# XChenZ/havatar

Hardware: AMD Instinct MI355X
Metric: rendered frames/sec @512^2, 64 samples/ray (higher is better)
Workload: dtype f32 emulated, full-width operands: every operand = hi + lo fp16 + tail (= the fp32 value itself, >= 24 significant bits); the three leading partial products on v_mfma_f32_32x32x16_f16, the three terms of order 2^-22 (hi.tail, tail.hi, lo.lo) on block-scaled 4-/6-bit v_mfma_scale_f32_32x32x64_f8f6f4

## Files before the change

### havatar_amd/_lib.py

```python
import ctypes as C
import os

from . import switches

_HERE = os.path.dirname(os.path.abspath(__file__))
LIB_PATH = os.path.join(_HERE, "lib", "libhavatar_hip.so")

HAV_F32, HAV_F16, HAV_BF16, HAV_F64 = 0, 1, 2, 3
HAV_MLP_SPLIT_BF16, HAV_MLP_F32, HAV_MLP_SPLIT_F16, HAV_MLP_SPLIT_F16_MX = 0, 1, 2, 3
ABI_VERSION = 8
HAV_FLAG_PAIR_KERNEL, HAV_FLAG_FINE_CACHE, HAV_FLAG_FINE_RECOMPUTE, HAV_FLAG_NO_FP16_GUARD = 1, 2, 4, 8
HAV_STATUS_FP16_FALLBACK = 1


class HavRenderParams(C.Structure):
    _fields_ = [("B", C.c_int32), ("R", C.c_int32), ("ray_stride", C.c_int32), ("S_c", C.c_int32),
                ("S_f", C.c_int32), ("perturb", C.c_int32), ("noise_std", C.c_float),
                ("plane_res", C.c_int32), ("plane_ch", C.c_int32), ("vol_res", C.c_int32),
                ("nerf_scale", C.c_float * 3), ("nerf_trans", C.c_float * 3),
                ("skin_scale", C.c_float * 3), ("skin_trans", C.c_float * 3),
                ("seed", C.c_uint64), ("rng_offset", C.c_uint64), ("mlp_mode", C.c_int32), ("flags", C.c_int32),
                ("rng_counter", C.c_void_p), ("workspace", C.c_void_p), ("workspace_bytes", C.c_uint64),
                ("dbg_zfine", C.c_void_p), ("status", C.c_void_p), ("grid_blocks", C.c_int32), ("reserved0", C.c_int32)]

# ... 65 lines not shown
    L.hav_triplane_gather_bwd.restype = i32
    L.hav_field_inputs_fwd.argtypes = [vp, C.POINTER(HavFieldParams), vp, vp, vp, vp, vp]
    L.hav_field_inputs_fwd.restype = i32
    L.hav_field_inputs_fwd_bf16.argtypes = [vp, C.POINTER(HavFieldParams), vp, vp, vp, vp, vp]
    L.hav_field_inputs_fwd_bf16.restype = i32
    L.hav_field_inputs_bwd.argtypes = [vp, vp, vp, C.POINTER(HavFieldParams), vp, vp, vp, vp, vp]
    L.hav_field_inputs_bwd.restype = i32
    L.hav_field_inputs_bwd_rows.argtypes = [vp, vp, vp, C.POINTER(HavFieldParams), vp, vp, vp, vp, i32, vp]
    L.hav_field_inputs_bwd_rows.restype = i32
    L.hav_field_inputs_bwd_fixed.argtypes = [vp, vp, vp, vp, vp, C.POINTER(HavFieldParams), vp, vp, vp, vp, vp]
    L.hav_field_inputs_bwd_fixed.restype = i32
    L.hav_field_inputs_bwd_fixed_scratch_bytes.argtypes = [C.POINTER(HavFieldParams)]
    L.hav_field_inputs_bwd_fixed_scratch_bytes.restype = i64
    L.hav_composite_fwd.argtypes = [vp] * 9 + [i64, i32, i32, i32, vp]
    L.hav_composite_fwd.restype = i32
    L.hav_composite_bwd.argtypes = [vp] * 10 + [i64, i32, i32, i32, vp]
    L.hav_composite_bwd.restype = i32
    for name, args in (("hav_composite_long_fwd", [vp] * 9 + [i64, i32, i32, i32, vp]),
                       ("hav_composite_long_bwd", [vp] * 10 + [i64, i32, i32, i32, vp]),
                       ("hav_composite_long_bwd_form", [vp] * 10 + [i64, i32, i32, i32, i32, vp]),
                       ("hav_haar_down2", [vp] * 5 + [f32, i32, i32, i32, i32, vp]),
                       ("hav_s2_image_loss_blocks", [i32, i32]),
                       ("hav_s2_image_loss_fwd", [vp, vp, vp] + [i64] * 4 + [vp] + [i64] * 3 + [vp] * 4 + [i32, i32, i32, vp]),
                       ("hav_s2_image_loss_bwd", [vp, vp] + [i64] * 4 + [vp, vp, vp] + [i64] * 4 + [vp] + [i64] * 3 + [vp] * 4
                        + [i32, i32, i32, i32, vp]),
                       ("hav_lpips_head_blocks", [i32] * 4),
                       ("hav_lpips_head_fwd", [vp] * 5 + [i32] * 4 + [vp]),
                       ("hav_lpips_head_bwd", [vp] * 6 + [i32] * 4 + [vp]),
                       ("hav_relu_mask_bwd", [vp] * 4 + [i32, i32, i64, vp]),
                       ("hav_image_metrics_blocks", [i32] * 4),
                       ("hav_image_metrics_f32", [vp] * 5 + [i32] * 4 + [f32, vp]),
                       ("hav_image_metrics_u8", [vp] * 5 + [i32] * 3 + [vp]),
                       ("hav_ssim_grad_blocks", [i32] * 4),
                       ("hav_ssim_loss_bwd_f32", [vp] * 5 + [i32] * 4 + [f32, vp])):
        try:
            fn = getattr(L, name)
        except AttributeError:
            raise HavatarLibraryError(f"{path} does not export {name}: it was built from older sources; rebuild it with "
                                      "`python -m havatar_amd.build --force`") from None
        fn.argtypes, fn.restype = args, (i64 if name.endswith("_blocks") else i32)
    L.hav_resample_depths.argtypes = [vp] * 5 + [i64, i32, i32, vp]
    L.hav_resample_depths.restype = i32
    L.hav_equal_linear_fwd.argtypes = [vp] * 4 + [C.c_float, C.c_float, i32, i32, i32, vp]
    L.hav_equal_linear_fwd.restype = i32
    L.hav_equal_linear_bwd.argtypes = [vp] * 6 + [C.c_float, C.c_float, i32, i32, i32, vp]
    L.hav_equal_linear_bwd.restype = i32
    L.hav_mlp_blob_bytes.restype = i64
    L.hav_mlp_pack.argtypes = [vp, C.POINTER(HavMlpWeights), vp]
    L.hav_mlp_pack.restype = i32
    for fn in (L.hav_haar_dwt, L.hav_haar_idwt):
        fn.argtypes = [vp, vp, vp, i32, i32, i32, i32, vp]
        fn.restype = i32
    L.hav_style_mlp.argtypes = [vp, vp, vp, i32, i32, i32, i32, f32, f32, vp]
    L.hav_style_mlp.restype = i32
    L.hav_haar_up2.argtypes = [vp, vp, vp, vp, vp, i32, i32, i32, i32, vp]
    L.hav_haar_up2.restype = i32
    L.hav_conv3x3_wgrad_scratch_bytes.argtypes = [i32] * 5
    L.hav_conv3x3_wgrad_scratch_bytes.restype = i64
    L.hav_conv3x3_wgrad.argtypes = [vp, vp, vp, vp, vp, vp, i32, i32, i32, i32, i32, vp]
    L.hav_conv3x3_wgrad.restype = i32
    L.hav_gemm_packed_bytes.argtypes = [i32, i32]
    L.hav_gemm_packed_bytes.restype = i64
    L.hav_gemm_pack.argtypes = [vp, vp, i32, i32, f32, vp]
    L.hav_gemm_pack.restype = i32
    L.hav_gemm_split.argtypes = [vp, vp, vp, vp, vp, i32, i32, i32, i32, vp]
    L.hav_gemm_split.restype = i32
    L.hav_upconv_finish.argtypes = [vp] * 7 + [f32, f32, i32, i32, i32, i32, i32, i32, vp]
# ... 106 lines not shown
```

### havatar_amd/build.py

```python
import os
import subprocess
import sys

from . import switches

HERE = os.path.dirname(os.path.abspath(__file__))
CSRC = os.path.join(HERE, "csrc")
LIBDIR = os.path.join(HERE, "lib")
LIB = os.path.join(LIBDIR, "libhavatar_hip.so")
SOURCES = ["hav_ops.hip", "hav_render.hip", "hav_train.hip", "hav_mlp_train.hip", "hav_conv.hip", "hav_conv3d.hip", "hav_decoder.hip",
           "hav_composite_long.hip", "hav_stage2.hip", "hav_s2_loss.hip", "hav_lpips.hip", "hav_metrics.hip", "hav_ssim_loss.hip"]
HEADERS = ["hav_common.h", os.path.join("..", "..", "include", "havatar.h")]
FLAGS = ["--offload-arch=gfx950", "-O3", "-std=c++17", "-fPIC", "-Wall", "-Wno-unused-function", "-Wno-unused-variable"]
BUILD_INFO = os.path.join(LIBDIR, "BUILD_INFO.json")
TESTED_HIPCC = ("HIP version: 7.2.26015-fc0010cf6a",
                "AMD clang version 22.0.0git (https://github.com/RadeonOpenCompute/llvm-project roc-7.2.0 26014 7b800a19466229b8479a78de19143dc33c3ab9b5)")


def hipcc_version(hipcc):
    out = subprocess.run([hipcc, "--version"], stdout=subprocess.PIPE, stderr=subprocess.STDOUT, check=False).stdout.decode(errors="replace")
    return tuple(ln.strip() for ln in out.splitlines()[:2])


def check_compiler(hipcc):
    ver = hipcc_version(hipcc)
    tested = ver == TESTED_HIPCC
    if not tested:
        msg = ("hipcc differs from the compiler this library's kernels were validated with:\n  found  %s\n  tested %s\n"
               "Re-run tools/stress_production.py and the -m gpu determinism tests on a GPU with the new build." % (ver, TESTED_HIPCC))
        if switches.off("HAVATAR_REQUIRE_TESTED_HIPCC"):
            raise RuntimeError(msg)
        import warnings
        warnings.warn(msg, RuntimeWarning, stacklevel=2)
    return ver, tested


def _stale():
    if not os.path.exists(LIB):
        return True
    t = os.path.getmtime(LIB)
    return any(os.path.getmtime(os.path.join(CSRC, f)) > t for f in SOURCES + HEADERS)


def build_info():
    import json
# ... 38 lines not shown
```

### havatar_amd/csrc/hav_render.hip

```cpp
#include "hav_common.h"
#include <stdio.h>
#include <stdlib.h>
#include <string.h>
#include <atomic>

#define HAV_HID 128
#define HAV_PC 64
#define HAV_IN (2 * HAV_PC + 48)
#define KPE_STEPS 24
#define K2_STEPS (HAV_HID / 2)
#define OFF_W1PE 0
#define OFF_W2 (OFF_W1PE + KPE_STEPS * 4 * 64)
#define OFF_W4 (OFF_W2 + K2_STEPS * 4 * 64)
#define OFF_WFT (OFF_W4 + K2_STEPS * 2 * 4)
#define LDS_FLOATS (OFF_WFT + HAV_HID * 64)
#define OFF_B1 LDS_FLOATS
#define OFF_B2 (OFF_B1 + 128)
#define OFF_B4 (OFF_B2 + 128)
#define OFF_BF (OFF_B4 + 4)
#define OFF_W1F (OFF_BF + 64)
#define OFF_WFF (OFF_W1F + 2 * 128 * 64)
#define OFF_A1S (OFF_WFF + K2_STEPS * 2 * 64)
#define OFF_A2S (OFF_A1S + 3 * 4 * 3 * 64 * 4)
#define OFF_W4S (OFF_A2S + 8 * 4 * 3 * 64 * 4)
#define LDS3_FLOATS (3 * 4 * 3 * 64 * 4 + 8 * 4 * 3 * 64 * 4 + K2_STEPS * 2 * 4)
#define OFF_A1H (OFF_W4S + K2_STEPS * 2 * 4)
#define OFF_A2H (OFF_A1H + 3 * 4 * 2 * 64 * 4)
#define OFF_W4H (OFF_A2H + 8 * 4 * 2 * 64 * 4)
#define OFF_AFH (OFF_W4H + K2_STEPS * 2 * 4)
#define HAV_TAPPAIR 1
#define HAV_TG 2
#define HAV_TG1 2
#define LDSH_FLOATS (3 * 4 * 2 * 64 * 4 + 8 * 4 * 2 * 64 * 4 + K2_STEPS * 2 * 4 + 8 * 2 * 2 * 64 * 4)
// ... 328 lines not shown

static bool attr_done(std::atomic<unsigned long long>& mask, int& dev)
{
    dev = 0;
    if (hipGetDevice(&dev) != hipSuccess || dev < 0 || dev > 63) dev = 0;
    return (mask.load(std::memory_order_acquire) >> dev) & 1ull;
}

extern "C" int hav_triplane_prepare(float* dst, const float* src_nchw, const void* mlp_blob, int B, int C, int H, int W,
                                    void* stream)
{
    if (!dst || !src_nchw || !mlp_blob || B < 1 || H < 1 || W < 1) return HAV_EINVAL;
    if (C != HAV_PC || (W & ((1 << HAV_TG) - 1)) || (W & ((1 << HAV_TG1) - 1))) return HAV_EUNSUP;
    const int HW = H * W;
    const size_t lds = (64 * 64 + 128 * 65 + 64 * 129) * sizeof(float);
    static std::atomic<unsigned long long> attr_mask{0};
    int dev;
    if (!attr_done(attr_mask, dev)) {
        hipError_t e = hipFuncSetAttribute((const void*)plane_project_kernel, hipFuncAttributeMaxDynamicSharedMemorySize, (int)lds);
        if (e != hipSuccess) return (int)e;
        attr_mask.fetch_or(1ull << dev, std::memory_order_release);
    }
    unsigned int* trailer = reinterpret_cast<unsigned int*>(dst + (size_t)2 * B * HW * 128);
    hipError_t me = hipMemsetAsync(trailer, 0, PREP_TRAILER_WORDS * 4, (hipStream_t)stream);
    if (me != hipSuccess) return (int)me;
    hipLaunchKernelGGL(plane_project_kernel, dim3((HW + 63) / 64, 2 * B), dim3(256), lds, (hipStream_t)stream, dst, src_nchw,
                       (const float*)mlp_blob, HW, trailer);
    HAV_LAUNCH_CHECK();
    hipLaunchKernelGGL(range_verdict_kernel, dim3(1), dim3(128), 0, (hipStream_t)stream, trailer, (const float*)mlp_blob);
    HAV_LAUNCH_CHECK();
    return 0;
}

#define DPP_QUAD_XOR1 0xB1
#define DPP_QUAD_XOR2 0x4E
#define DPP_ROW_SHR(n) (0x110 + (n))
#define DPP_ROW_MIRROR 0x140
#define DPP_ROW_HALF_MIRROR 0x141

template <int CTRL> __device__ __forceinline__ float dpp_mov(float old, float v)
{
    return __int_as_float(__builtin_amdgcn_update_dpp(__float_as_int(old), __float_as_int(v), CTRL, 0xf, 0xf, false));
}
__device__ __forceinline__ float row16_sum(float v)
{
    v += dpp_mov<DPP_QUAD_XOR1>(0.f, v);
    v += dpp_mov<DPP_QUAD_XOR2>(0.f, v);
    v += dpp_mov<DPP_ROW_HALF_MIRROR>(0.f, v);
    v += dpp_mov<DPP_ROW_MIRROR>(0.f, v);
    return v;
}
__device__ __forceinline__ float row16_max(float v)
{
    v = fmaxf(v, dpp_mov<DPP_QUAD_XOR1>(0.f, v));
    v = fmaxf(v, dpp_mov<DPP_QUAD_XOR2>(0.f, v));
    v = fmaxf(v, dpp_mov<DPP_ROW_HALF_MIRROR>(0.f, v));
    v = fmaxf(v, dpp_mov<DPP_ROW_MIRROR>(0.f, v));
    return v;
}
__device__ __forceinline__ float row16_scan_mul(float v)
{
    v *= dpp_mov<DPP_ROW_SHR(1)>(1.f, v);
    v *= dpp_mov<DPP_ROW_SHR(2)>(1.f, v);
    v *= dpp_mov<DPP_ROW_SHR(4)>(1.f, v);
    v *= dpp_mov<DPP_ROW_SHR(8)>(1.f, v);
    return v;
// ... 1723 lines not shown
```

### havatar_amd/model/nerf_model.py

```python
import logging

import torch
import torch.nn as nn

from .network.embedder import get_embedder
from .styleUnet import StyleGAN_zxc
from .. import switches
from ..utils.sh_util import eval_sh
from ..utils.util import create_UniformBoxWarp, sample_from_triplane_new

_MLP_MODE_LOGGED = False


class _SplitKLinear(torch.autograd.Function):

    @staticmethod
    def forward(ctx, x, weight, bias):
        ctx.save_for_backward(x, weight)
        ctx.has_bias = bias is not None
        return torch.nn.functional.linear(x, weight, bias)

    @staticmethod
    def backward(ctx, dy):
        x, weight = ctx.saved_tensors
# ... 16 lines not shown
    return layer(x)


class ConditionalTriplaneNeRFModel_multiRender_split_view(nn.Module):
    def __init__(self, XYZ_bounding, num_encoding_fn_xyz=8, latent_code_dim=32, triPlane_feat_dim=32, rgb_feat_dim=32,
                 triplane_res=256, use_emb=True, enc_mode="split", sh_deg=2, cond_latent=True, cond_c_dim=0):
        super().__init__()
        if enc_mode != "split":
            raise NotImplementedError("only enc_mode='split' is on the hot path (model/nerf_trainer.py:19-26)")
        self.name = "ConditionalTriplaneNeRFModel_multiRender_split_view"
        self.pos_embedder, self.dim_xyz = get_embedder(multires=num_encoding_fn_xyz, input_dims=3, include_input=False)
        self.sh_deg = sh_deg
        self.use_sh = sh_deg >= 1
        include_xyz = self.dim_xyz if use_emb else 0
        self.dim_latent_code = 0 if cond_latent else latent_code_dim
        self.triPlane_feat_dim = triPlane_feat_dim
        self.rgb_feat_dim = rgb_feat_dim * (sh_deg + 1) ** 2
        self.use_emb, self.cond_latent, self.cond_c_dim = use_emb, cond_latent, cond_c_dim
        self.shared_backbone = self.two_head = False
        enc = dict(out_ch=triPlane_feat_dim, out_size=triplane_res, style_dim=latent_code_dim, middle_size=16, zero_latent=False,
                   zero_noise=True, no_skip=True, n_mlp=4, inp_size=256)
        self.XY_gen = StyleGAN_zxc(inp_ch=7, **enc)
        self.YZ_gen = StyleGAN_zxc(inp_ch=13, **enc)
        self.gridwarper = create_UniformBoxWarp(XYZ_bounding)
        self.layers_xyz = nn.ModuleList([nn.Linear(2 * triPlane_feat_dim + self.dim_latent_code + include_xyz, 128), nn.Linear(128, 128)])
        self.fc_alpha = nn.Linear(128, 1)
        self.fc_rgbFeat = nn.Linear(128, 64)
        self.fc_rgb = nn.Linear(64, self.rgb_feat_dim)
        self.relu = torch.nn.functional.relu
        self.triPlane_embeddings = None
        if not cond_latent:
            self.register_buffer("zero_latent", torch.zeros(latent_code_dim, dtype=torch.float32).reshape(1, -1))

    def set_conditional_embedding(self, **cond):
        styles = None
        if "latents" in cond:
            lat = cond["latents"]
            c = cond["cond_c"].reshape(lat.shape[0], -1)
            if self.cond_latent:
                styles = [torch.cat([lat, c], -1)] if self.cond_c_dim > 0 else [lat]
            else:
                styles = [self.zero_latent.expand(lat.shape[0], -1)]
        front, right = cond["front_render_cond"], cond["right_render_cond"]
        left = cond["left_render_cond"].flip(dims=[3])
        if left.shape[1] > 3:
            left = left[:, :-1]
        yz_in = torch.cat([left, right], dim=1)
        if front.is_cuda and not torch.is_grad_enabled() and switches.on("HAVATAR_ENC_STREAMS"):
            cur = torch.cuda.current_stream(front.device)
            side = self.__dict__.get("_side_stream")
            if side is None or side.device != front.device:
                side = self.__dict__["_side_stream"] = torch.cuda.Stream(device=front.device)
            side.wait_stream(cur)
            with torch.cuda.stream(side):
                yz, _ = self.YZ_gen(styles, yz_in)
            xy, _ = self.XY_gen(styles, front)
            cur.wait_stream(side)
            yz.record_stream(cur)
        else:
            xy, _ = self.XY_gen(styles, front)
            yz, _ = self.YZ_gen(styles, yz_in)
        self.triPlane_embeddings = torch.stack([xy, yz], dim=0)

    def sample_pts_triplane_feat(self, batch_pts, bidx=None):
        q = self.gridwarper(batch_pts)
        planes = self.triPlane_embeddings if bidx is None else self.triPlane_embeddings[:, bidx]
        if q.is_cuda and q.dtype == torch.float32 and q.ndim == 3 and planes.ndim == 5 and planes.shape[0] == 2 \
                and switches.on("HAVATAR_HIP_GATHER"):
            from ..native.gather import triplane_gather
            return triplane_gather(q, planes)
        f = sample_from_triplane_new(q, planes, padding_mode="zeros")
        return f.reshape(-1, f.shape[-1] * f.shape[-2])

    def forward(self, inp, pts_feat):
        xyz, dirs = inp[..., :3], inp[..., 3:]
        return self.mlp(torch.cat([pts_feat, self.pos_embedder(xyz)], -1), dirs)

    def mlp(self, x, dirs=None):
        if (x.is_cuda and x.dtype == torch.float32 and x.ndim == 2 and x.shape[1] == 176 and self.sh_deg == 0 and x.shape[0] >= 1024
                and torch.is_grad_enabled() and switches.choice("HAVATAR_TRAIN_MLP") == "bf16"):
            from ..native import mlp_train
            ws = self.mlp_tensors()
            if [tuple(w.shape) for w in ws] == mlp_train._SHAPES:
                global _MLP_MODE_LOGGED
                if not _MLP_MODE_LOGGED:
                    _MLP_MODE_LOGGED = True
                    logging.getLogger("havatar_amd").info(
                        "radiance MLP under autograd: bf16-operand MFMA node (HAVATAR_TRAIN_MLP=bf16; parameter gradients in the 2e-2 "
                        "class of fp32 nn.Linear) -- HAVATAR_TRAIN_MLP=torch keeps the reference's fp32 layers")
                return mlp_train.fused_mlp(x, ws)
        for layer in self.layers_xyz:
            x = self.relu(_linear(layer, x))
        alpha = _linear(self.fc_alpha, x)
        x = _linear(self.fc_rgbFeat, x)
# ... 9 lines not shown
```

### havatar_amd/model/nerf_trainer.py

```python
import numpy as np
import torch
from einops import rearrange

from . import nerf_model
from .. import switches
from .Skinning_Field import Deformation_Field_new
from ..render import RayMarcher
from ..utils.nerf_util import sample_pdf, volume_render_radiance_field
from ..utils.training_util import get_minibatches
from ..utils.util import UniformBoxWarp_new, get_box_warp_param


_warned_wide_sampling = False


def _warn_wide_sampling(widest):
    global _warned_wide_sampling
    if _warned_wide_sampling:
        return
    _warned_wide_sampling = True
    import warnings
    warnings.warn("training with %d samples in a pass: the native compositing kernels hold 64, so this step takes the ATen statement of "
                  "the whole march.  Set HAVATAR_COMPOSITE_LONG=1 to keep it on the native route (up to 128 samples per pass)." % widest,
                  RuntimeWarning, stacklevel=3)


class Trainer(torch.nn.Module):
    def __init__(self, cfg, latent_codes_size=0, freeze_motion=True):
        super().__init__()
        self.cfg = cfg
        e = cfg.experiment
        self.latent_codes = torch.nn.Parameter(torch.zeros(latent_codes_size, e.latent_code_dim)) if latent_codes_size > 0 else None
        self.model_mode = e.model_mode
        latent_code_dim = e.latent_code_dim + (12 if e.cond_pose else 0) + (52 if e.cond_expr else 0)
        bounding = cfg.models.coarse.XYZ_bounding
        self.model_coarse = nerf_model.ConditionalTriplaneNeRFModel_multiRender_split_view(
            XYZ_bounding=bounding, triPlane_feat_dim=64, rgb_feat_dim=3, triplane_res=128, sh_deg=0,
            latent_code_dim=latent_code_dim, cond_c_dim=latent_code_dim - e.latent_code_dim)
        self.render_size, self.gen_size = cfg.models.StyleUnet.inp_size, cfg.models.StyleUnet.out_size
        b = {k: np.asarray(v, dtype=np.float64).copy() for k, v in zip("XYZ", bounding)}
        b["Y"][0] = 0.3 * b["Y"][1]
        scales, trans = get_box_warp_param(b["X"], b["Y"], b["Z"])
        self.headpose_skin_net = Deformation_Field_new(gridwarper=UniformBoxWarp_new(scales=scales, trans=trans))
        if freeze_motion:
            self.headpose_skin_net.requires_grad = False
        self._marcher = None

    def _hip_marcher(self):
        if self._marcher is None:
            gw, sw = self.model_coarse.gridwarper, self.headpose_skin_net.gridwarper
            f = lambda t: t.detach().reshape(3).cpu().tolist()
            self._marcher = RayMarcher(f(gw.scale_factor), f(gw.trans_factor), f(sw.scale_factor), f(sw.trans_factor))
        return self._marcher

    def nerf_forward(self, **inputs):
        cond_c = inputs["inv_head_T"].view(inputs["inv_head_T"].shape[0], -1)
        self.model_coarse.set_conditional_embedding(
            front_render_cond=inputs["front_render_cond"], left_render_cond=inputs["left_render_cond"],
            right_render_cond=inputs["right_render_cond"], latents=inputs["latent_code"], cond_c=cond_c)
        self._planes_dirty = True
        inv_head_T, ray_batch, background_prior = inputs["inv_head_T"], inputs["ray_batch"], inputs["background_prior"]
        mode = inputs["mode"]
        opt = getattr(self.cfg.nerf, mode)
        rd = ray_batch[..., 3:6]
        restore = [rd.shape[:-1] + (-1,), rd.shape[:-1], rd.shape[:-1], rd.shape[:-1]]
        if opt.num_fine > 0:
            restore += restore[:-1]
        if ray_batch.is_cuda:
            rays = ray_batch
        else:
            viewdirs = rd / rd.norm(p=2, dim=-1).unsqueeze(-1)
            rays = torch.cat((ray_batch, viewdirs), dim=-1)
        if self._use_hip(rays):
            self._decline_coarse = bool(inputs.get("_fine_maps_only", False)) and opt.num_fine > 0
            out = list(self.predict_and_render_radiance(mode, rays, background_prior, inv_head_T=inv_head_T))
            self._decline_coarse = False
        else:
            if rays.is_cuda:
                cap = max(switches.integer("HAVATAR_TRAIN_CHUNK_RAYS"), opt.chunksize)
                chunk = min(rays.shape[1], max(cap // rays.shape[0], 1))
            else:
                chunk = opt.chunksize // rays.shape[0]
            rb = get_minibatches(rays, chunksize=chunk, dim=1)
            bg = get_minibatches(background_prior, chunksize=chunk, dim=1) if background_prior is not None else None
            pred = [self.predict_and_render_radiance(mode, r, None if bg is None else bg[i], inv_head_T=inv_head_T) for i, r in enumerate(rb)]
            out = [torch.cat(im, dim=1) if im[0] is not None else None for im in zip(*pred)]
        if mode == "validation":
            out = [im.view(shape) if im is not None else None for im, shape in zip(out, restore)]
            return tuple(out) if opt.num_fine > 0 else tuple(out + [None, None, None])[:7]
        return tuple(out)

    def forward(self, **data):
        ray_batch, background_prior = data["ray_batch"], data["background_prior"]
# ... 11 lines not shown
            mask = acc_fine if acc_fine is not None else acc_coarse
            render = render.reshape(B, self.render_size, self.render_size, -1).permute(0, 3, 1, 2)
            mask = mask.reshape(B, self.render_size, self.render_size, -1).permute(0, 3, 1, 2)
            return render, mask, latent_code_loss
        return rgb_coarse, _, acc_coarse, weights, rgb_fine, _, acc_fine, latent_code_loss

    def _latent_code_loss(self, latent_code, mode):
        lc = self.latent_codes
        if mode != "train" and lc.is_cuda and not torch.is_grad_enabled():
            from ..graph import weights_epoch
            key = (lc.data_ptr(), lc._version, weights_epoch())
            hit = self.__dict__.get("_lc_loss")
            if hit is None or hit[0] != key:
                hit = self.__dict__["_lc_loss"] = (key, torch.square(latent_code - lc.mean(dim=0, keepdims=True).detach()).mean())
            return hit[1]
        return torch.square(latent_code - lc.mean(dim=0, keepdims=True).detach()).mean()

    def _use_hip(self, ray_batch):
        if not ray_batch.is_cuda:
            return False
        if not torch.is_grad_enabled():
            return True
        planes = getattr(self.model_coarse, "triPlane_embeddings", None)
        if ray_batch.requires_grad or (planes is not None and planes.requires_grad):
            return False
        return not any(p.requires_grad for p in self.parameters())

    def predict_and_render_radiance(self, mode, ray_batch, background_prior, inv_head_T):
        opt = getattr(self.cfg.nerf, mode)
        if self._use_hip(ray_batch):
            return self._render_hip(opt, ray_batch, background_prior, inv_head_T)
        return self._render_torch(opt, ray_batch, background_prior, inv_head_T)

    def _render_hip(self, opt, ray_batch, background_prior, inv_head_T):
        m = self._hip_marcher()
        m.set_mlp(*[t.detach() for t in self.model_coarse.mlp_tensors()])
        planes = self.model_coarse.triPlane_embeddings
        key = (planes.data_ptr(), planes._version, m._blob_key)
        if getattr(self, "_planes_dirty", True) or getattr(self, "_planes_key", None) != key:
            m.set_triplane(planes.detach())
            self._planes_key, self._planes_dirty = key, False
        vol = self.headpose_skin_net.current_volume().detach()
        return m.render(ray_batch, background_prior, inv_head_T, vol, int(opt.num_coarse), int(opt.num_fine),
                        perturb=bool(opt.perturb), noise_std=float(opt.radiance_field_noise_std),
                        coarse_outputs=not getattr(self, "_decline_coarse", False))

    def _render_torch(self, opt, ray_batch, background_prior, inv_head_T):
        B, R = ray_batch.shape[:2]
        ro, rd = ray_batch[..., :3], ray_batch[..., 3:6]
        near, far = ray_batch[..., 6:7], ray_batch[..., 7:8]
        t = torch.linspace(0.0, 1.0, opt.num_coarse, dtype=ro.dtype, device=ro.device)
        z = near * (1.0 - t) + far * t
        if opt.perturb:
            mids = 0.5 * (z[..., 1:] + z[..., :-1])
            upper, lower = torch.cat((mids, z[..., -1:]), dim=-1), torch.cat((z[..., :1], mids), dim=-1)
            z = lower + (upper - lower) * torch.rand(z.shape, dtype=ro.dtype, device=ro.device)
        bg = background_prior.reshape(-1, background_prior.shape[-1]) if background_prior is not None else None

        widest = max(opt.num_coarse, opt.num_coarse // 2 + opt.num_coarse % 2 + opt.num_fine)
        fused = (ro.is_cuda and ro.dtype == torch.float32 and self.model_coarse.sh_deg == 0 and switches.on("HAVATAR_HIP_TRAIN"))
        if fused and widest > 64:
            from ..native.train_ops import composite_long_enabled
            long_on = composite_long_enabled()
            if not long_on and 64 < widest <= 128:
                _warn_wide_sampling(widest)
            fused = long_on and widest <= 128
# ... 60 lines not shown
```

### havatar_amd/model/styleUnet.py

```python
import math
import random

import torch
from torch import nn
from torch.nn import functional as F

from .op import FusedLeakyReLU, conv2d_gradfix, fused_leaky_relu, upfirdn2d
from .. import switches
from ..graph import weights_epoch
from ..native import conv as _conv


def _fused_conv_enabled():
    return switches.on("HAVATAR_FUSED_CONV")


def _hip_train():
    return switches.on("HAVATAR_HIP_TRAIN")


def _conv_s2():
    return switches.on("HAVATAR_CONV_S2")


# ... 628 lines not shown
        if no_skip:
            self.conv_out = ConvLayer(ch[out_size], out_ch, 1)
        else:
            self.to_rgb1 = ToRGB(ch[middle_size], self.style_dim, out_channel=out_ch * 4, upsample=False, use_wt=False)
        self.num_layers = (self.log_size - self.middle_log_size) * 2 + 1
        for li in range(self.num_layers):
            res = (li + 8) // 2
            self.noises.register_buffer(f"noise_{li}", torch.randn(1, 1, 2 ** res, 2 ** res))
        in_channel = ch[middle_size]
        for i in range(self.middle_log_size + 1, self.log_size + 1):
            out_channel = ch[2 ** i]
            self.convs.append(StyledConv(in_channel, out_channel, 3, self.style_dim, upsample=True, blur_kernel=blur_kernel))
            self.convs.append(StyledConv(out_channel, out_channel, 3, self.style_dim, blur_kernel=blur_kernel))
            self.to_rgbs.append(None if no_skip else ToRGB(out_channel, self.style_dim, out_channel=out_ch * 4, use_wt=False))
            in_channel = out_channel
        self.n_latent = self.log_size * 2 - (self.middle_log_size * 2 - 1) + 1 if n_latent is None else n_latent
        self.zero_noise = self.make_noise(zero_noise=True) if zero_noise else None
        if zero_latent:
            self.register_buffer("zero_latents", torch.zeros(1, self.n_latent, self.style_dim))
        else:
            self.zero_latents = None

    def make_noise(self, zero_noise=False):
        fn = torch.zeros if zero_noise else torch.randn
        noises = [torch.randn(1, 1, 2 ** self.middle_log_size, 2 ** self.middle_log_size)]
        for i in range(self.middle_log_size + 1, self.log_size + 1):
            noises += [fn(1, 1, 2 ** i, 2 ** i), fn(1, 1, 2 ** i, 2 ** i)]
        return noises

    def get_latent(self, styles, n_latent=None, inject_index=None):
        return _mix_latents([_run_style(self.style, s) for s in styles], self.n_latent if n_latent is None else n_latent, inject_index)

    def forward(self, styles, cond_feats, return_latents=False, inject_index=None, truncation=1, truncation_latent=None,
                input_is_latent=False, noise=None, randomize_noise=True, **kwargs):
        B = cond_feats.shape[0]
        if self.zero_latents is None:
            if not input_is_latent:
                assert self.n_mlp > 0
                styles = [_run_style(self.style, s) for s in styles]
            if truncation < 1:
                styles = [truncation_latent + truncation * (s - truncation_latent) for s in styles]
            latent = _mix_latents(styles, self.n_latent, inject_index)
        else:
            latent = self.zero_latents.expand(B, -1, -1)
        if self.zero_noise is not None:
            noise = [n.to(cond_feats.device) for n in self.zero_noise]
            self.zero_noise = noise
        elif noise is None:
            noise = [None] * self.num_layers if randomize_noise else [getattr(self.noises, f"noise_{i}") for i in range(self.num_layers)]

        pairs = [(self.conv1.conv, 0)] + ([] if self.no_skip else [(self.to_rgb1.conv, 1)])
        for k in range(len(self.convs) // 2):
            pairs += [(self.convs[2 * k].conv, 1 + 2 * k), (self.convs[2 * k + 1].conv, 2 + 2 * k)]
            if not self.no_skip:
                pairs.append((self.to_rgbs[k].conv, 3 + 2 * k))
        _prefetch_styles(self, pairs, latent)
        cond_list = self._encode(cond_feats)
        out = self.conv1(self.input(latent), latent[:, 0], noise=noise[0])
        skip = None if self.no_skip else self.to_rgb1(out, latent[:, 1])
        i = 1
        for conv_a, conv_b, n_a, n_b, to_rgb in zip(self.convs[::2], self.convs[1::2], noise[1::2], noise[2::2], self.to_rgbs):
            if 1 < i <= 2 * len(cond_list) + 1:
                out = self.comb_convs[-(i // 2)](torch.cat([out, cond_list[-(i // 2)]], dim=1))
            out = conv_b(conv_a(out, latent[:, i], noise=n_a), latent[:, i + 1], noise=n_b)
            if not self.no_skip:
                skip = to_rgb(out, latent[:, i + 2], skip)
            i += 2
        image = self.conv_out(out) if self.no_skip else skip
        return (image, latent) if return_latents else (image, None)


class SWGAN_unet(nn.Module, _CondEncoder):

    def __init__(self, inp_size, inp_ch, out_ch, out_size, style_dim, n_mlp, middle_size=8, c_dim=0, channel_multiplier=2,
                 blur_kernel=(1, 3, 3, 1), lr_mlp=0.01):
        super().__init__()
        self.inp_size, self.style_dim = inp_size, style_dim
        self.middle_log_size = int(math.log(middle_size, 2))
        self.style = _style_mlp(style_dim + c_dim, style_dim, n_mlp, lr_mlp)
        self.channels = ch = _CHANNELS(channel_multiplier)
        self.log_size = int(math.log(out_size, 2)) - 1

        in_channel = ch[inp_size // 2]
        self.from_rgbs, self.cond_convs, self.comb_convs = nn.ModuleList(), nn.ModuleList(), nn.ModuleList()
        self.comb_convs.append(ConvLayer(in_channel * 2, in_channel, 3))
        self.conv_in = ConvLayer(inp_ch, in_channel, 3, downsample=True)
        for i in range(int(math.log(inp_size, 2)) - 2, self.middle_log_size - 1, -1):
            out_channel = ch[2 ** i]
            self.from_rgbs.append(FromRGB(in_channel, inp_ch, downsample=True, use_wt=False))
            self.cond_convs.append(ConvBlock(in_channel, out_channel, blur_kernel))
            self.comb_convs.append(ConvLayer(out_channel * 2 if i > self.middle_log_size else out_channel, out_channel, 3))
            in_channel = out_channel

        self.convs, self.to_rgbs, self.noises = nn.ModuleList(), nn.ModuleList(), nn.Module()
        self.num_layers = (self.log_size - self.middle_log_size) * 2
        for li in range(self.num_layers):
            res = (li + 8) // 2
            self.noises.register_buffer(f"noise_{li}", torch.randn(1, 1, 2 ** res, 2 ** res))
        in_channel = ch[middle_size]
        for i in range(self.middle_log_size + 1, self.log_size + 1):
            out_channel = ch[2 ** i]
            self.convs.append(StyledConv(in_channel, out_channel, 3, style_dim, upsample=True, blur_kernel=blur_kernel))
# ... 52 lines not shown
```

### havatar_amd/render.py

```python
import ctypes as C

import torch

from . import _lib, switches
from .graph import weights_epoch

_DEBUG_SYNC = switches.off("HAVATAR_DEBUG_SYNC")


def _ptr(t):
    return None if t is None else C.c_void_p(t.data_ptr())


def _stream():
    return C.c_void_p(torch.cuda.current_stream().cuda_stream)


def _chk_f32_cuda(name, t, allow_none=False):
    if t is None:
        if allow_none:
            return None
        raise RuntimeError(f"{name} is required")
    if not t.is_cuda:
        raise RuntimeError(f"{name} must be a CUDA/HIP tensor")
# ... 32 lines not shown
        self.last_variant = None

    def set_mlp(self, W1, b1, W2, b2, Wa, ba, Wf, bf, Wc, bc, force=False):
        ts = [_chk_f32_cuda(n, t) for n, t in zip(("W1", "b1", "W2", "b2", "Wa", "ba", "Wf", "bf", "Wc", "bc"),
                                                   (W1, b1, W2, b2, Wa, ba, Wf, bf, Wc, bc))]
        key = tuple((t.data_ptr(), t._version) for t in ts) + (weights_epoch(),)
        if not force and key == self._blob_key and self.blob is not None:
            return
        L = _lib.lib()
        if self.blob is None or self.blob.device != ts[0].device:
            self.blob = torch.empty(int(L.hav_mlp_blob_bytes()) // 4, dtype=torch.float32, device=ts[0].device)
        w = _lib.HavMlpWeights(*[t.data_ptr() for t in ts])
        with torch.cuda.device(ts[0].device):
            _lib.check(L.hav_mlp_pack(_ptr(self.blob), C.byref(w), _stream()), "hav_mlp_pack")
        self._blob_key = key
        self._keep = ts

    def set_triplane(self, planes_nchw):
        if self.blob is None:
            raise RuntimeError("set_mlp() must be called before set_triplane()")
        p = _chk_f32_cuda("triPlane_embeddings", planes_nchw)
        two, B, Cc, H, W = p.shape
        if two != 2 or Cc != self.plane_ch or H != W:
            raise RuntimeError(f"unsupported tri-plane shape {tuple(p.shape)}")
        self.plane_res = H
        need = int(_lib.lib().hav_triplane_prepared_bytes(B, H, W)) // 4
        if self.planes_cl is None or self.planes_cl.numel() != need or self.planes_cl.device != p.device:
            self.planes_cl = torch.empty(need, dtype=torch.float32, device=p.device)
        self._planes_B = B
        with torch.cuda.device(p.device):
            _lib.check(_lib.lib().hav_triplane_prepare(_ptr(self.planes_cl), _ptr(p), _ptr(self.blob), B, Cc, H, W, _stream()),
                       "hav_triplane_prepare")
        self._planes_key = self._blob_key

    def render(self, rays, bg, inv_T, skin_vol, S_c, S_f, perturb=False, noise_std=0.0,
               t_rand=None, u_rand=None, noise_c=None, noise_f=None, dbg_zfine=False, coarse_outputs=True):
        if self.blob is None or self.planes_cl is None:
            raise RuntimeError("set_mlp() and set_triplane() must be called before render()")
        if self._planes_key != self._blob_key:
            raise RuntimeError("weights changed since set_triplane(): call set_triplane() again")
        rays = _chk_f32_cuda("ray_batch", rays)
        B, R, stride = rays.shape
        bg = _chk_f32_cuda("background_prior", bg, allow_none=True)
        inv_T = _chk_f32_cuda("inv_head_T", inv_T)
        vol = _chk_f32_cuda("canonical_W", skin_vol)
        if vol.dim() == 5:
            vol = vol[0]
        if self._planes_B != B or inv_T.shape[0] != B:
            raise RuntimeError("batch mismatch between rays, inv_head_T and the tri-plane")
        dev = rays.device
        S_fp = (S_c + 1) // 2 + S_f if S_f > 0 else 0
        p = _lib.HavRenderParams()
        p.B, p.R, p.ray_stride, p.S_c, p.S_f = B, R, stride, S_c, S_f
        p.perturb, p.noise_std = int(bool(perturb)), float(noise_std)
        p.plane_res, p.plane_ch, p.vol_res = self.plane_res, self.plane_ch, vol.shape[-1]
        for i in range(3):
            p.nerf_scale[i], p.nerf_trans[i] = self.nerf_scale[i], self.nerf_trans[i]
            p.skin_scale[i], p.skin_trans[i] = self.skin_scale[i], self.skin_trans[i]
        p.seed, p.rng_offset = self.seed, self.rng_offset
        p.mlp_mode, p.flags = self.mlp_mode, self.flags
        p.grid_blocks = int(self.grid_blocks)
        if self._status is None or self._status.device != dev:
            self._status = torch.zeros(1, dtype=torch.int32, device=dev)
        p.status = self._status.data_ptr()
        if self.rng_counter is None or self.rng_counter.device != dev:
            self.rng_counter = torch.zeros(1, dtype=torch.int64, device=dev)
# ... 90 lines not shown
```

### include/havatar.h

```cpp
#ifndef HAVATAR_H
#define HAVATAR_H

#include <stdint.h>

#ifdef __cplusplus
extern "C" {
#endif

#define HAV_ABI_VERSION 8

#define HAV_EINVAL   (-1)
#define HAV_EUNSUP   (-2)

#define HAV_F32  0
#define HAV_F16  1
#define HAV_BF16 2
#define HAV_F64  3

int hav_abi_version(void);

int hav_fused_bias_act(void* out, const void* x, const void* b, const void* ref,
                       int dtype, int act, int grad, float alpha, float scale,
                       int64_t size_x, int64_t step_b, int64_t size_b, void* stream);

// ... 215 lines not shown
    int32_t  reserved0;
} HavRenderParams;

#define HAV_FLAG_PAIR_KERNEL     1
#define HAV_FLAG_FINE_CACHE      2
#define HAV_FLAG_FINE_RECOMPUTE  4
#define HAV_FLAG_NO_FP16_GUARD   8
#define HAV_FLAGS_ALL           15

#define HAV_STATUS_FP16_FALLBACK 1u

#define HAV_MLP_SPLIT_BF16 0
#define HAV_MLP_F32        1
#define HAV_MLP_SPLIT_F16_MX 3
#define HAV_MLP_SPLIT_F16  2

int64_t hav_render_workspace_bytes(const HavRenderParams* p);

typedef struct HavMlpWeights {
    const float* W1; const float* b1;
    const float* W2; const float* b2;
    const float* Wa; const float* ba;
    const float* Wf; const float* bf;
    const float* Wc; const float* bc;
} HavMlpWeights;

int64_t hav_mlp_blob_bytes(void);
int hav_mlp_pack(void* blob, const HavMlpWeights* w, void* stream);

int64_t hav_triplane_prepared_bytes(int B, int H, int W);
int hav_triplane_prepare(float* dst, const float* src_nchw, const void* mlp_blob, int B, int C, int H, int W,
                         void* stream);

typedef struct HavRenderOut {
    float* rgb_coarse;
    float* depth_coarse;
    float* acc_coarse;
    float* weights_max;
    float* rgb_fine;
    float* depth_fine;
    float* acc_fine;
} HavRenderOut;

int hav_render_rays(const HavRenderParams* p, const float* rays, const float* bg,
                    const float* inv_T, const float* planes_prepared, const float* skin_vol,
                    const void* mlp_blob, const float* t_rand, const float* u_rand,
                    const float* noise_c, const float* noise_f, const HavRenderOut* out,
                    void* stream);

int hav_debug_mlp_layer(float* y, const float* x, const void* mlp_blob, int mlp_mode, int layer, int64_t n, void* stream);

int hav_render_variant_name(const HavRenderParams* p, int coarse_outputs, int injected_rand, char* buf, int len);

int hav_gen_rays(float* rays, int H, int W, const float intr[4], const float c2w[12],
                 float near, float far, int y0, int y1, void* stream);

#ifdef __cplusplus
}
#endif
#endif
```

Measured before the change: 114.2.

## Fuse tri-plane conv_out 1x1 conv with tri-plane preparation into one handoff kernel

Adds a HIP kernel that computes the StyleUNet conv_out 1x1 convolution plus FusedLeakyReLU for both XY and YZ generators, writes the planes, and in the same pass projects them through the MLP first-layer weights into the prepared layout with range-check trailer. This replaces the separate conv_out, torch.stack, and hav_triplane_prepare launches, saving intermediate round trips through memory and several kernel launches per frame. The generator forward gains a features_only mode, and the encoder call is moved earlier. It adds a new ABI entry and code path limited to inference with 64 plane channels, with fallback to the old path otherwise.

Result: no change. 115.1, median of 6 (+0.8%).

```diff
diff --git a/havatar_amd/_lib.py b/havatar_amd/_lib.py
--- a/havatar_amd/_lib.py
+++ b/havatar_amd/_lib.py
@@ -121,7 +121,8 @@
                        ("hav_image_metrics_f32", [vp] * 5 + [i32] * 4 + [f32, vp]),
                        ("hav_image_metrics_u8", [vp] * 5 + [i32] * 3 + [vp]),
                        ("hav_ssim_grad_blocks", [i32] * 4),
-                       ("hav_ssim_loss_bwd_f32", [vp] * 5 + [i32] * 4 + [f32, vp])):
+                       ("hav_ssim_loss_bwd_f32", [vp] * 5 + [i32] * 4 + [f32, vp]),
+                       ("hav_planes_handoff", [vp] * 8 + [f32] * 4 + [vp] + [i32] * 5 + [vp])):
         try:
             fn = getattr(L, name)
         except AttributeError:
diff --git a/havatar_amd/build.py b/havatar_amd/build.py
--- a/havatar_amd/build.py
+++ b/havatar_amd/build.py
@@ -9,8 +9,8 @@
 LIBDIR = os.path.join(HERE, "lib")
 LIB = os.path.join(LIBDIR, "libhavatar_hip.so")
 SOURCES = ["hav_ops.hip", "hav_render.hip", "hav_train.hip", "hav_mlp_train.hip", "hav_conv.hip", "hav_conv3d.hip", "hav_decoder.hip",
-           "hav_composite_long.hip", "hav_stage2.hip", "hav_s2_loss.hip", "hav_lpips.hip", "hav_metrics.hip", "hav_ssim_loss.hip"]
-HEADERS = ["hav_common.h", os.path.join("..", "..", "include", "havatar.h")]
+           "hav_composite_long.hip", "hav_stage2.hip", "hav_s2_loss.hip", "hav_lpips.hip", "hav_metrics.hip", "hav_ssim_loss.hip", "hav_frame_ends.hip"]
+HEADERS = ["hav_common.h", "hav_prep_layout.h", os.path.join("..", "..", "include", "havatar.h")]
 FLAGS = ["--offload-arch=gfx950", "-O3", "-std=c++17", "-fPIC", "-Wall", "-Wno-unused-function", "-Wno-unused-variable"]
 BUILD_INFO = os.path.join(LIBDIR, "BUILD_INFO.json")
 TESTED_HIPCC = ("HIP version: 7.2.26015-fc0010cf6a",
diff --git a/havatar_amd/csrc/hav_frame_ends.hip b/havatar_amd/csrc/hav_frame_ends.hip
--- /dev/null
+++ b/havatar_amd/csrc/hav_frame_ends.hip
@@ -0,0 +1,169 @@
+#include "hav_common.h"
+#include "hav_prep_layout.h"
+#include <atomic>
+
+#define FE_T 128
+#define FE_KC 32
+#define FE_YS 132
+#define FE_LDS_FLOATS (64 * FE_YS + 64 * FE_YS + FE_KC * FE_T + FE_KC * 64 + 128)
+
+struct HandoffSide {
+    const float* x;
+    const float* wt;
+    const float* bias;
+    float slope, gain;
+};
+
+__global__ void __launch_bounds__(512) planes_handoff_kernel(float* __restrict__ planes, float* __restrict__ prep, HandoffSide s0,
+                                                             HandoffSide s1, const float* __restrict__ w1f, int B, int Cin, int HW,
+                                                             unsigned int* __restrict__ trailer)
+{
+    extern __shared__ __attribute__((aligned(16))) float sm[];
+    float* sY = sm;
+    float* sW1 = sY + 64 * FE_YS;
+    float* sX = sW1 + 64 * FE_YS;
+    float* sW = sX + FE_KC * FE_T;
+    unsigned int* sMax = reinterpret_cast<unsigned int*>(sW + FE_KC * 64);
+    const int tid = threadIdx.x;
+    const int pb = blockIdx.y;
+    const int p = pb / B, b = pb - p * B;
+    const int t0 = blockIdx.x * FE_T;
+    const HandoffSide S = p ? s1 : s0;
+    const float* xsrc = S.x + (size_t)b * Cin * HW;
+    const int g = tid >> 4, q = tid & 15;
+    const bool live = t0 + 4 * g < HW;
+
+    const int xr = tid >> 5, xc = (tid & 31) * 4;
+    const bool xin = t0 + xc < HW;
+    float4 px0, px1, pw;
+    auto fetch = [&](int kc) {
+        const float* xa = xsrc + (size_t)(kc * FE_KC + xr) * HW + t0 + xc;
+        px0 = xin ? *reinterpret_cast<const float4*>(xa) : make_float4(0.f, 0.f, 0.f, 0.f);
+        px1 = xin ? *reinterpret_cast<const float4*>(xa + (size_t)16 * HW) : make_float4(0.f, 0.f, 0.f, 0.f);
+        pw = *reinterpret_cast<const float4*>(S.wt + (size_t)kc * FE_KC * 64 + 4 * tid);
+    };
+    fetch(0);
+    if (tid < 128) sMax[tid] = 0u;
+    {
+        const float* wsrc = w1f + (size_t)p * 128 * 64;
+        for (int i = tid; i < 128 * 64; i += 512) sW1[(i & 63) * FE_YS + (i >> 6)] = wsrc[i];
+    }
+
+    float acc[4][4], tot[4][4];
+#pragma unroll
+    for (int j = 0; j < 4; ++j)
+#pragma unroll
+        for (int i = 0; i < 4; ++i) tot[j][i] = 0.f;
+    const int nk = Cin / FE_KC;
+    for (int kc = 0; kc < nk; ++kc) {
+#pragma unroll
+        for (int j = 0; j < 4; ++j)
+#pragma unroll
+            for (int i = 0; i < 4; ++i) acc[j][i] = 0.f;
+        __syncthreads();
+        *reinterpret_cast<float4*>(sX + xr * FE_T + xc) = px0;
+        *reinterpret_cast<float4*>(sX + (xr + 16) * FE_T + xc) = px1;
+        *reinterpret_cast<float4*>(sW + 4 * tid) = pw;
+        __syncthreads();
+        if (kc + 1 < nk) fetch(kc + 1);
+#pragma unroll 8
+        for (int k = 0; k < FE_KC; ++k) {
+            const float4 xv = *reinterpret_cast<const float4*>(sX + k * FE_T + 4 * g);
+            const float4 wv = *reinterpret_cast<const float4*>(sW + k * 64 + 4 * q);
+            const float xs[4] = {xv.x, xv.y, xv.z, xv.w}, ws[4] = {wv.x, wv.y, wv.z, wv.w};
+#pragma unroll
+            for (int j = 0; j < 4; ++j)
+#pragma unroll
+                for (int i = 0; i < 4; ++i) acc[j][i] = fmaf(ws[j], xs[i], acc[j][i]);
+        }
+#pragma unroll
+        for (int j = 0; j < 4; ++j)
+#pragma unroll
+            for (int i = 0; i < 4; ++i) tot[j][i] += acc[j][i];
+    }
+#pragma unroll
+    for (int j = 0; j < 4; ++j) {
+        const float bv = S.bias ? S.bias[4 * q + j] : 0.f;
+        float y[4];
+#pragma unroll
+        for (int i = 0; i < 4; ++i) {
+            const float v = tot[j][i] + bv;
+            y[i] = (v > 0.f ? v : v * S.slope) * S.gain;
+        }
+        *reinterpret_cast<float4*>(sY + (4 * q + j) * FE_YS + 4 * g) = make_float4(y[0], y[1], y[2], y[3]);
+    }
+    __syncthreads();
+    {
+        float* dst = planes + (size_t)pb * 64 * HW;
+        for (int i = tid; i < 64 * (FE_T / 4); i += 512) {
+            const int co = i >> 5, c4 = (i & 31) * 4;
+            if (t0 + c4 < HW) *reinterpret_cast<float4*>(dst + (size_t)co * HW + t0 + c4) = *reinterpret_cast<const float4*>(sY + co * FE_YS + c4);
+        }
+    }
+    if (live) {
+        float pa[8][4];
+#pragma unroll
+        for (int o = 0; o < 8; ++o)
+#pragma unroll
+            for (int i = 0; i < 4; ++i) pa[o][i] = 0.f;
+#pragma unroll 4
+        for (int c = 0; c < 64; ++c) {
+            const float4 yv = *reinterpret_cast<const float4*>(sY + c * FE_YS + 4 * g);
+            const float4 wa = *reinterpret_cast<const float4*>(sW1 + c * FE_YS + 8 * q);
+            const float4 wb = *reinterpret_cast<const float4*>(sW1 + c * FE_YS + 8 * q + 4);
+            const float ys[4] = {yv.x, yv.y, yv.z, yv.w}, ws[8] = {wa.x, wa.y, wa.z, wa.w, wb.x, wb.y, wb.z, wb.w};
+#pragma unroll
+            for (int o = 0; o < 8; ++o)
+#pragma unroll
+                for (int i = 0; i < 4; ++i) pa[o][i] = fmaf(ws[o], ys[i], pa[o][i]);
+        }
+        float4* out = reinterpret_cast<float4*>(prep + (size_t)pb * HW * 128 + (size_t)((t0 >> 2) + g) * 512 + q * 32);
+#pragma unroll
+        for (int h = 0; h < 2; ++h)
+#pragma unroll
+            for (int i = 0; i < 4; ++i) out[h * 4 + i] = make_float4(pa[4 * h][i], pa[4 * h + 1][i], pa[4 * h + 2][i], pa[4 * h + 3][i]);
+#pragma unroll
+        for (int o = 0; o < 8; ++o) {
+            float m = 0.f;
+            unsigned int bad = 0;
+#pragma unroll
+            for (int i = 0; i < 4; ++i) {
+                const float a = fabsf(pa[o][i]);
+                bad |= (a != a);
+                m = fmaxf(m, a);
+            }
+            atomicMax(&sMax[8 * q + o], bad ? 0x7FC00000u : __float_as_uint(m));
+        }
+    }
+    __syncthreads();
+    if (tid < 128) atomicMax(&trailer[p * 128 + tid], sMax[tid]);
+}
+
+extern "C" int hav_planes_handoff(float* planes_nchw, float* prepared, const float* x0, const float* x1, const float* wt0,
+                                  const float* wt1, const float* bias0, const float* bias1, float slope0, float gain0, float slope1,
+                                  float gain1, const void* mlp_blob, int B, int Cin, int Cout, int H, int W, void* stream)
+{
+    if (!planes_nchw || !prepared || !x0 || !x1 || !wt0 || !wt1 || !mlp_blob || B < 1 || Cin < 1 || H < 1 || W < 1) return HAV_EINVAL;
+    const HavPrepLayout L = hav_prep_layout();
+    if (Cout != L.plane_ch || L.plane_ch != 64 || L.tg0 != 2 || L.tg1 != 2 || (Cin % FE_KC) || (W & 3)) return HAV_EUNSUP;
+    if ((int64_t)H * W > (int64_t)1 << 24 || (int64_t)2 * B > 65535) return HAV_EUNSUP;
+    if (((uintptr_t)planes_nchw | (uintptr_t)prepared | (uintptr_t)x0 | (uintptr_t)x1 | (uintptr_t)wt0 | (uintptr_t)wt1) & 15) return HAV_EINVAL;
+    const int HW = H * W;
+    const size_t lds = FE_LDS_FLOATS * sizeof(float);
+    static std::atomic<unsigned long long> attr_mask{0};
+    int dev = 0;
+    if (hipGetDevice(&dev) != hipSuccess || dev < 0 || dev > 63) dev = 0;
+    if (!((attr_mask.load(std::memory_order_acquire) >> dev) & 1ull)) {
+        hipError_t e = hipFuncSetAttribute((const void*)planes_handoff_kernel, hipFuncAttributeMaxDynamicSharedMemorySize, (int)lds);
+        if (e != hipSuccess) return (int)e;
+        attr_mask.fetch_or(1ull << dev, std::memory_order_release);
+    }
+    unsigned int* trailer = reinterpret_cast<unsigned int*>(prepared + (size_t)2 * B * HW * 128);
+    hipError_t me = hipMemsetAsync(trailer, 0, (size_t)L.trailer_words * 4, (hipStream_t)stream);
+    if (me != hipSuccess) return (int)me;
+    const HandoffSide s0 = {x0, wt0, bias0, slope0, gain0}, s1 = {x1, wt1, bias1, slope1, gain1};
+    hipLaunchKernelGGL(planes_handoff_kernel, dim3((HW + FE_T - 1) / FE_T, 2 * B), dim3(512), lds, (hipStream_t)stream, planes_nchw,
+                       prepared, s0, s1, (const float*)mlp_blob + L.off_w1f, B, Cin, HW, trailer);
+    HAV_LAUNCH_CHECK();
+    return hav_prep_verdict_launch(trailer, mlp_blob, (hipStream_t)stream);
+}
diff --git a/havatar_amd/csrc/hav_prep_layout.h b/havatar_amd/csrc/hav_prep_layout.h
--- /dev/null
+++ b/havatar_amd/csrc/hav_prep_layout.h
@@ -0,0 +1,12 @@
+#pragma once
+#include <hip/hip_runtime.h>
+
+struct HavPrepLayout {
+    int off_w1f;
+    int plane_ch;
+    int tg0, tg1;
+    int trailer_words;
+};
+
+__attribute__((visibility("hidden"))) HavPrepLayout hav_prep_layout();
+__attribute__((visibility("hidden"))) int hav_prep_verdict_launch(unsigned int* trailer, const void* mlp_blob, hipStream_t stream);
diff --git a/havatar_amd/csrc/hav_render.hip b/havatar_amd/csrc/hav_render.hip
--- a/havatar_amd/csrc/hav_render.hip
+++ b/havatar_amd/csrc/hav_render.hip
@@ -1,4 +1,5 @@
 #include "hav_common.h"
+#include "hav_prep_layout.h"
 #include <stdio.h>
 #include <stdlib.h>
 #include <string.h>
@@ -393,6 +394,14 @@
     return 0;
 }
 
+HavPrepLayout hav_prep_layout() { return HavPrepLayout{OFF_W1F, HAV_PC, HAV_TG, HAV_TG1, PREP_TRAILER_WORDS}; }
+int hav_prep_verdict_launch(unsigned int* trailer, const void* mlp_blob, hipStream_t stream)
+{
+    hipLaunchKernelGGL(range_verdict_kernel, dim3(1), dim3(128), 0, stream, trailer, (const float*)mlp_blob);
+    HAV_LAUNCH_CHECK();
+    return 0;
+}
+
 #define DPP_QUAD_XOR1 0xB1
 #define DPP_QUAD_XOR2 0x4E
 #define DPP_ROW_SHR(n) (0x110 + (n))
diff --git a/havatar_amd/model/nerf_model.py b/havatar_amd/model/nerf_model.py
--- a/havatar_amd/model/nerf_model.py
+++ b/havatar_amd/model/nerf_model.py
@@ -72,7 +72,7 @@
         if not cond_latent:
             self.register_buffer("zero_latent", torch.zeros(latent_code_dim, dtype=torch.float32).reshape(1, -1))
 
-    def set_conditional_embedding(self, **cond):
+    def set_conditional_embedding(self, handoff=None, **cond):
         styles = None
         if "latents" in cond:
             lat = cond["latents"]
@@ -86,6 +86,12 @@
         if left.shape[1] > 3:
             left = left[:, :-1]
         yz_in = torch.cat([left, right], dim=1)
+        sides = None
+        if handoff is not None and front.is_cuda and front.dtype == torch.float32 and not torch.is_grad_enabled():
+            sides = (self.XY_gen.conv_out_side(), self.YZ_gen.conv_out_side())
+            if sides[0] is None or sides[1] is None:
+                sides = None
+        gen_kw = {"features_only": True} if sides is not None else {}
         if front.is_cuda and not torch.is_grad_enabled() and switches.on("HAVATAR_ENC_STREAMS"):
             cur = torch.cuda.current_stream(front.device)
             side = self.__dict__.get("_side_stream")
@@ -93,13 +99,19 @@
                 side = self.__dict__["_side_stream"] = torch.cuda.Stream(device=front.device)
             side.wait_stream(cur)
             with torch.cuda.stream(side):
-                yz, _ = self.YZ_gen(styles, yz_in)
-            xy, _ = self.XY_gen(styles, front)
+                yz, _ = self.YZ_gen(styles, yz_in, **gen_kw)
+            xy, _ = self.XY_gen(styles, front, **gen_kw)
             cur.wait_stream(side)
             yz.record_stream(cur)
         else:
-            xy, _ = self.XY_gen(styles, front)
-            yz, _ = self.YZ_gen(styles, yz_in)
+            xy, _ = self.XY_gen(styles, front, **gen_kw)
+            yz, _ = self.YZ_gen(styles, yz_in, **gen_kw)
+        if sides is not None:
+            planes = handoff(xy, yz, sides[0], sides[1])
+            if planes is not None:
+                self.triPlane_embeddings = planes
+                return
+            xy, yz = self.XY_gen.conv_out(xy), self.YZ_gen.conv_out(yz)
         self.triPlane_embeddings = torch.stack([xy, yz], dim=0)
 
     def sample_pts_triplane_feat(self, batch_pts, bidx=None):
diff --git a/havatar_amd/model/nerf_trainer.py b/havatar_amd/model/nerf_trainer.py
--- a/havatar_amd/model/nerf_trainer.py
+++ b/havatar_amd/model/nerf_trainer.py
@@ -55,10 +55,11 @@
 
     def nerf_forward(self, **inputs):
         cond_c = inputs["inv_head_T"].view(inputs["inv_head_T"].shape[0], -1)
+        self._planes_dirty = True
         self.model_coarse.set_conditional_embedding(
+            handoff=self._planes_handoff if self._use_hip(inputs["ray_batch"]) else None,
             front_render_cond=inputs["front_render_cond"], left_render_cond=inputs["left_render_cond"],
             right_render_cond=inputs["right_render_cond"], latents=inputs["latent_code"], cond_c=cond_c)
-        self._planes_dirty = True
         inv_head_T, ray_batch, background_prior = inputs["inv_head_T"], inputs["ray_batch"], inputs["background_prior"]
         mode = inputs["mode"]
         opt = getattr(self.cfg.nerf, mode)
@@ -136,6 +137,16 @@
             return self._render_hip(opt, ray_batch, background_prior, inv_head_T)
         return self._render_torch(opt, ray_batch, background_prior, inv_head_T)
 
+    def _planes_handoff(self, xy_feat, yz_feat, xy_side, yz_side):
+        if torch.is_grad_enabled():
+            return None
+        m = self._hip_marcher()
+        m.set_mlp(*[t.detach() for t in self.model_coarse.mlp_tensors()])
+        planes = m.set_triplane_from_features(xy_feat, yz_feat, xy_side, yz_side)
+        if planes is not None:
+            self._planes_key, self._planes_dirty = (planes.data_ptr(), planes._version, m._blob_key), False
+        return planes
+
     def _render_hip(self, opt, ray_batch, background_prior, inv_head_T):
         m = self._hip_marcher()
         m.set_mlp(*[t.detach() for t in self.model_coarse.mlp_tensors()])
diff --git a/havatar_amd/model/styleUnet.py b/havatar_amd/model/styleUnet.py
--- a/havatar_amd/model/styleUnet.py
+++ b/havatar_amd/model/styleUnet.py
@@ -684,8 +684,9 @@
         return _mix_latents([_run_style(self.style, s) for s in styles], self.n_latent if n_latent is None else n_latent, inject_index)
 
     def forward(self, styles, cond_feats, return_latents=False, inject_index=None, truncation=1, truncation_latent=None,
-                input_is_latent=False, noise=None, randomize_noise=True, **kwargs):
+                input_is_latent=False, noise=None, randomize_noise=True, features_only=False, **kwargs):
         B = cond_feats.shape[0]
+        cond_list = self._encode(cond_feats)
         if self.zero_latents is None:
             if not input_is_latent:
                 assert self.n_mlp > 0
@@ -707,7 +708,6 @@
             if not self.no_skip:
                 pairs.append((self.to_rgbs[k].conv, 3 + 2 * k))
         _prefetch_styles(self, pairs, latent)
-        cond_list = self._encode(cond_feats)
         out = self.conv1(self.input(latent), latent[:, 0], noise=noise[0])
         skip = None if self.no_skip else self.to_rgb1(out, latent[:, 1])
         i = 1
@@ -718,8 +718,22 @@
             if not self.no_skip:
                 skip = to_rgb(out, latent[:, i + 2], skip)
             i += 2
-        image = self.conv_out(out) if self.no_skip else skip
+        if features_only and self.no_skip:
+            image = out
+        else:
+            image = self.conv_out(out) if self.no_skip else skip
         return (image, latent) if return_latents else (image, None)
+
+    def conv_out_side(self):
+        layer = getattr(self, "conv_out", None)
+        if layer is None or len(layer) != 2 or not isinstance(layer[0], EqualConv2d) or not isinstance(layer[1], FusedLeakyReLU):
+            return None
+        ec, act = layer[0], layer[1]
+        if ec.weight.shape[2:] != (1, 1) or ec.stride != 1 or ec.padding != 0 or ec.bias is not None:
+            return None
+        from ..native import frame_ends
+        wt = ec._cached("w1x1t", ec.weight, lambda: frame_ends.pack_conv_out(ec.weight, ec.scale))
+        return wt, act.bias, act.negative_slope, act.scale
 
 
 class SWGAN_unet(nn.Module, _CondEncoder):
diff --git a/havatar_amd/native/frame_ends.py b/havatar_amd/native/frame_ends.py
--- /dev/null
+++ b/havatar_amd/native/frame_ends.py
@@ -0,0 +1,45 @@
+import ctypes as C
+
+import torch
+
+from .. import _lib
+
+PLANE_CH = 64
+K_CHUNK = 32
+
+
+def _f32_hip(t, shape=None):
+    return (isinstance(t, torch.Tensor) and t.is_cuda and t.dtype == torch.float32 and t.is_contiguous()
+            and t.data_ptr() % 16 == 0 and (shape is None or tuple(t.shape) == tuple(shape)))
+
+
+def pack_conv_out(weight, scale):
+    return (weight.detach() * scale).reshape(weight.shape[0], weight.shape[1]).t().contiguous()
+
+
+def prepared_numel(B, H, W):
+    return int(_lib.lib().hav_triplane_prepared_bytes(B, H, W)) // 4
+
+
+def planes_handoff(x0, x1, side0, side1, blob, prepared):
+    if torch.is_grad_enabled() or not _f32_hip(x0) or x0.dim() != 4 or not _f32_hip(x1, x0.shape) or x1.device != x0.device:
+        return None
+    B, Cin, H, W = x0.shape
+    if B < 1 or Cin < K_CHUNK or Cin % K_CHUNK or W % 4 or H * W > 1 << 24 or 2 * B > 65535:
+        return None
+    for wt, bias, _, _ in (side0, side1):
+        if not _f32_hip(wt, (Cin, PLANE_CH)) or wt.device != x0.device:
+            return None
+        if bias is not None and not (_f32_hip(bias, (PLANE_CH,)) and bias.device == x0.device):
+            return None
+    if not (_f32_hip(blob) and blob.device == x0.device and _f32_hip(prepared) and prepared.device == x0.device
+            and prepared.numel() == prepared_numel(B, H, W)):
+        return None
+    planes = torch.empty(2, B, PLANE_CH, H, W, dtype=torch.float32, device=x0.device)
+    p = lambda t: None if t is None else C.c_void_p(t.data_ptr())
+    with torch.cuda.device(x0.device):
+        rc = _lib.lib().hav_planes_handoff(p(planes), p(prepared), p(x0), p(x1), p(side0[0]), p(side1[0]), p(side0[1]), p(side1[1]),
+                                           float(side0[2]), float(side0[3]), float(side1[2]), float(side1[3]), p(blob), B, Cin, PLANE_CH,
+                                           H, W, C.c_void_p(torch.cuda.current_stream().cuda_stream))
+    _lib.check(rc, "hav_planes_handoff")
+    return planes
diff --git a/havatar_amd/render.py b/havatar_amd/render.py
--- a/havatar_amd/render.py
+++ b/havatar_amd/render.py
@@ -88,6 +88,24 @@
             _lib.check(_lib.lib().hav_triplane_prepare(_ptr(self.planes_cl), _ptr(p), _ptr(self.blob), B, Cc, H, W, _stream()),
                        "hav_triplane_prepare")
         self._planes_key = self._blob_key
+
+    def set_triplane_from_features(self, xy_feat, yz_feat, xy_side, yz_side):
+        from .native import frame_ends
+        if self.blob is None or not isinstance(xy_feat, torch.Tensor) or xy_feat.dim() != 4 or not xy_feat.is_cuda:
+            return None
+        B, _, H, W = xy_feat.shape
+        if H != W or xy_side[0].shape[-1] != self.plane_ch or self.blob.device != xy_feat.device:
+            return None
+        need = frame_ends.prepared_numel(B, H, W)
+        buf = self.planes_cl
+        if buf is None or buf.numel() != need or buf.device != xy_feat.device:
+            buf = torch.empty(need, dtype=torch.float32, device=xy_feat.device)
+        planes = frame_ends.planes_handoff(xy_feat, yz_feat, xy_side, yz_side, self.blob, buf)
+        if planes is None:
+            return None
+        self.planes_cl, self.plane_res, self._planes_B = buf, H, B
+        self._planes_key = self._blob_key
+        return planes
 
     def render(self, rays, bg, inv_T, skin_vol, S_c, S_f, perturb=False, noise_std=0.0,
                t_rand=None, u_rand=None, noise_c=None, noise_f=None, dbg_zfine=False, coarse_outputs=True):
diff --git a/include/havatar.h b/include/havatar.h
--- a/include/havatar.h
+++ b/include/havatar.h
@@ -271,6 +271,10 @@
 int hav_triplane_prepare(float* dst, const float* src_nchw, const void* mlp_blob, int B, int C, int H, int W,
                          void* stream);
 
+int hav_planes_handoff(float* planes_nchw, float* prepared, const float* x0, const float* x1, const float* wt0, const float* wt1,
+                       const float* bias0, const float* bias1, float slope0, float gain0, float slope1, float gain1,
+                       const void* mlp_blob, int B, int Cin, int Cout, int H, int W, void* stream);
+
 typedef struct HavRenderOut {
     float* rgb_coarse;
     float* depth_coarse;
```
